# apapiu/transformer_latent_diffusion

Hardware: AMD Instinct MI355X
Metric: images/sec (256px, 35-step CFG sampling), denoiser only (higher is better)
Workload: dtype bf16; 1 GPU; C1: 100M-param denoiser (d=768, L=12), 32x32x4 latents, 35 steps + CFG 6, DPM-Solver++(2M), 64 images/GPU (model batch 128); images_per_gpu=64, global_batch=64, n_iter=35, parallelism=single GPU

## Files before the change

### transformer_latent_diffusion_amd/csrc/tld_common.h

```cpp
#pragma once
#include <hip/hip_runtime.h>
#include <atomic>
#include <mutex>
#include <stdint.h>
#include "tld_gemm_plan.h"

namespace tld {

typedef __attribute__((ext_vector_type(8))) __bf16 bf16x8;
typedef __attribute__((ext_vector_type(4))) __bf16 bf16x4;
typedef __attribute__((ext_vector_type(2))) __bf16 bf16x2;
typedef __attribute__((ext_vector_type(16))) float f32x16;
typedef __attribute__((ext_vector_type(4))) float f32x4;
typedef __attribute__((ext_vector_type(4))) unsigned u32x4;
typedef __attribute__((ext_vector_type(8))) int i32x8;
typedef __attribute__((ext_vector_type(2))) float f32x2;

constexpr int kWave = 64;
constexpr int kHeadDim = 64;
constexpr float kLnEps = 1e-5f;

template <int CTRL>
__device__ __forceinline__ float dpp_add(float v) {
    const int s = __builtin_amdgcn_update_dpp(0, __float_as_int(v), CTRL, 0xf, 0xf, true);
// ... 185 lines not shown
    std::mutex mu;
    template <class F> void run(int want, F&& set_attribute) {
        int dev = 0;
        (void)hipGetDevice(&dev);
        std::atomic<int>& a = v[dev & 63];
        if (a.load(std::memory_order_acquire) >= want) return;
        std::lock_guard<std::mutex> lk(mu);
        if (a.load(std::memory_order_relaxed) >= want) return;
        set_attribute();
        a.store(want, std::memory_order_release);
    }
};
inline int ptr_device(const void* p) {
    hipPointerAttribute_t a;
    if (p && hipPointerGetAttributes(&a, p) == hipSuccess) return a.device;
    (void)hipGetLastError();
    return -1;
}
struct PtrDeviceGuard {
    int prev = -1; bool switched = false;
    explicit PtrDeviceGuard(const void* p) {
        const int dev = ptr_device(p);
        if (dev >= 0 && hipGetDevice(&prev) == hipSuccess && prev != dev) switched = hipSetDevice(dev) == hipSuccess;
    }
    ~PtrDeviceGuard() { if (switched) (void)hipSetDevice(prev); }
    PtrDeviceGuard(const PtrDeviceGuard&) = delete;
    PtrDeviceGuard& operator=(const PtrDeviceGuard&) = delete;
};
inline int device_cu_count() {
    static int cus[64] = {0};
    int dev = 0;
    (void)hipGetDevice(&dev);
    int& c = cus[dev & 63];
    if (!c) {
        int n = 0;
        if (hipDeviceGetAttribute(&n, hipDeviceAttributeMultiprocessorCount, dev) != hipSuccess || n <= 0) n = 256;
        c = n;
    }
    return c;
}

enum : int {
    EP_EMBED_PLAIN = 0, EP_EMBED_MFMA = 1 , EP_LN_Q4 = 5 , EP_LN_GENERIC = 9, EP_LN_MX8 = 10,
    EP_QKV_ATTN = 11, EP_QKV_LN = 12, EP_QKV_PLAIN = 13,
    EP_ATT_256 = 14, EP_ATT_CHUNKED = 15, EP_ATT_64 = 17 , EP_ATT_MASKED = 19,
    EP_CROSS_MFMA = 20 , EP_CROSS_GPW1 = 24, EP_CROSS_GPWN = 25, EP_CROSS_VALU = 26, EP_CROSS_FANOUT = 27,
    EP_UP_FUSED16 = 28, EP_UP_FUSED32_SEAM = 29, EP_UP_FUSED16_SMALL = 30, EP_UP_PLAIN = 31, EP_DW_WHOLE = 32, EP_DW_TILED = 33, EP_DW_STREAM = 34,
    EP_DOWN_STATS = 35, EP_DOWN_NOSTATS = 36, EP_DOWN_MAIN = 37, EP_DOWN_SMALL64 = 38, EP_DOWN_SMALL128 = 39,
    EP_SPLITK4 = 40, EP_SPLITK8 = 41, EP_SPLITK_SMALL = 42, EP_SPLITK_FINISH12 = 43, EP_SPLITK_FINISH6 = 44,
    EP_TAIL_MFMA = 45 , EP_TAIL_PLAIN = 49, EP_UPDATE = 50, EP_UPDATE_FROM = 51, EP_UPDATE_FROM_MASK = 52, EP_START_MIX = 53,
    EP_QUANT_MX8 = 54, EP_CROSS_F8 = 55, EP_DW_TILED_F8 = 56, EP_DW_STREAM_F8 = 57,
    EP_UPDATE_REQ = 58, EP_UPDATE_REQ_MASK = 59, EP_START_MIX_REQ = 60,
    EP_TAIL_FOLD = 16,
    EP_COUNT = 61
};
extern thread_local uint64_t* g_path_sink;
inline void note_path(int bit) { if (g_path_sink) *g_path_sink |= 1ull << bit; }

int launch_gemm(const GemmParams& p, int epilogue, hipStream_t s);
void launch_updw_pp(const GemmParams& p, const GemmPlan& plan, hipStream_t s);
void launch_splitk_pp(const GemmParams& p, const GemmPlan& plan, hipStream_t s);
void launch_down_pp(const GemmParams& p, const GemmPlan& plan, hipStream_t s);
void launch_dwconv_seam(const uint32_t* seam, const uint32_t* dw_wpk, const float* dw_b_half, bf16* out, int ldo, int batch, int channels, hipStream_t s);
void launch_gemm_tn(const GemmParams& p, hipStream_t s);

void set_last_error(const char* msg);

void launch_quant_mx8(const bf16* in, uint8_t* out, uint8_t* scale, int M, int K, hipStream_t s);
void quant_mx8_host(const float* w, int rows, int K, uint8_t* out, uint8_t* scale);

void launch_attention(const bf16* qk, const bf16* vt, bf16* att, int batch, int ntok, int heads,
                      hipStream_t s);

void launch_dwconv_gelu(const bf16* in, bf16* out, const float* w9c , const float* bias, const float* w9c_half,
                        const float* bias_half, int batch, int grid, int channels, hipStream_t s, uint8_t* out8 = nullptr,
                        uint8_t* scale8 = nullptr);

struct EmbedParams {
    const float* x;
    const float* conv_w;
    const float* conv_b;
    const float* ln1_w; const float* ln1_b;
    const float* lin_wt;
    const bf16* lin_w_hl;
    const float* lin_b;
    const float* ln2_w; const float* ln2_b;
    const float* pos;
    resid_t* tok;
    float2* stats_out;
    int batch, src_batch;
    const int* src_row;
    int C, S, p, grid, pd, d, ntok;
};
void launch_embed(const EmbedParams& p, hipStream_t s);

void launch_layernorm_bf16(const resid_t* x, const float* g, const float* b, bf16* out, int M, int d,
                           hipStream_t s);
bool layernorm_mx8_supported(int d);
void launch_layernorm_mx8(const resid_t* x, const float* g, const float* b, uint8_t* out8, uint8_t* scale8, int M, int d,
                          hipStream_t s);

struct CrossRowParams {
    resid_t* x;
    const resid_t* x_in;
    const bf16* att;
    int src_batch;
// ... 76 lines not shown
```

### transformer_latent_diffusion_amd/csrc/tld_cond.hip

```cpp
#include "tld_common.h"
#include <hip/hip_fp16.h>

namespace tld {

namespace {

__global__ void sinusoid_kernel(const float* __restrict__ sigma, const float* __restrict__ angular,
                                float* __restrict__ out, int T, int half) {
    const int i = blockIdx.x * blockDim.x + threadIdx.x;
    if (i >= T * half) return;
    const int t = i / half, k = i - t * half;
    const float ph = angular[k] * sigma[t];
    out[(size_t)t * 2 * half + k] = sinf(ph);
    out[(size_t)t * 2 * half + half + k] = cosf(ph);
}

constexpr int LR = 8;
__global__ __launch_bounds__(256) void linear_f32_kernel(const float* __restrict__ in, int ldi,
                                                         const float* __restrict__ W,
                                                         const float* const* __restrict__ Wl,
                                                         const float* __restrict__ bias,
                                                         float* __restrict__ out, size_t out_lstride, int ldo, int T,
                                                         int K, int N, int act) {
    if (Wl) { W = Wl[blockIdx.z]; out += (size_t)blockIdx.z * out_lstride; }
    extern __shared__ __attribute__((aligned(16))) char smem[];
    float* xs = reinterpret_cast<float*>(smem);
    const int t0 = blockIdx.y * LR;
    for (int i = threadIdx.x; i < LR * K; i += 256) {
        const int r = i / K, k = i - r * K;
        const int t = t0 + r;
        xs[i] = t < T ? in[(size_t)t * ldi + k] : 0.f;
    }
    __syncthreads();
    const int lane = threadIdx.x & 63, wid = threadIdx.x >> 6;
    for (int c = 0; c < 16; ++c) {
        const int n = blockIdx.x * 64 + wid * 16 + c;
        if (n >= N) break;
        float acc[LR];
#pragma unroll
        for (int r = 0; r < LR; ++r) acc[r] = 0.f;
        const float* wrow = W + (size_t)n * K;
        for (int k = lane; k < K; k += 64) {
            const float w = wrow[k];
#pragma unroll
            for (int r = 0; r < LR; ++r) acc[r] += xs[r * K + k] * w;
        }
#pragma unroll
        for (int r = 0; r < LR; ++r) acc[r] = wave_sum(acc[r]);
        if (lane < LR) {
            float v = 0.f;
#pragma unroll
            for (int r = 0; r < LR; ++r) if (lane == r) v = acc[r];
            const int t = t0 + lane;
            if (t < T) {
                v += bias ? bias[n] : 0.f;
                if (act == 1) v = gelu_erf(v);
                out[(size_t)t * ldo + n] = v;
            }
        }
    }
}

__global__ __launch_bounds__(256) void layernorm_f32_kernel(const float* __restrict__ x,
                                                            const float* __restrict__ g,
                                                            const float* __restrict__ b,
                                                            float* __restrict__ out, int M, int d) {
    const int lane = threadIdx.x & 63;
    const int row = blockIdx.x * 4 + (threadIdx.x >> 6);
    if (row >= M) return;
    float s = 0.f;
    for (int k = lane; k < d; k += 64) s += x[(size_t)row * d + k];
    const float mean = wave_sum(s) / (float)d;
    float q = 0.f;
    for (int k = lane; k < d; k += 64) { const float c = x[(size_t)row * d + k] - mean; q += c * c; }
    const float rstd = 1.0f / sqrtf(wave_sum(q) / (float)d + kLnEps);
    for (int k = lane; k < d; k += 64)
        out[(size_t)row * d + k] = (x[(size_t)row * d + k] - mean) * rstd * g[k] + b[k];
}

__global__ __launch_bounds__(256) void wq_kernel(const float* __restrict__ kmat, size_t k_lstride, int ldk,
                                                 const float* const* __restrict__ Wql,
                                                 const float* const* __restrict__ gammal,
                                                 const float* const* __restrict__ betal, float* __restrict__ wq,
                                                 size_t wq_lstride, float* __restrict__ bwq, size_t bwq_lstride, int T,
                                                 int H, int d) {
    const float* __restrict__ Wq = Wql[blockIdx.z];
    const float* __restrict__ gamma = gammal[blockIdx.z];
    const float* __restrict__ beta = betal[blockIdx.z];
    kmat += (size_t)blockIdx.z * k_lstride; wq += (size_t)blockIdx.z * wq_lstride; bwq += (size_t)blockIdx.z * bwq_lstride;
    __shared__ float ks[LR][64];
    __shared__ float red[4][LR];
    const int h = blockIdx.x, t0 = blockIdx.y * LR;
    for (int i = threadIdx.x; i < LR * 64; i += 256) {
        const int r = i >> 6, c = i & 63;
        const int t = t0 + r;
        ks[r][c] = t < T ? kmat[(size_t)t * ldk + h * 64 + c] * 0.125f : 0.f;
    }
    __syncthreads();
    float bacc[LR];
#pragma unroll
    for (int r = 0; r < LR; ++r) bacc[r] = 0.f;
    for (int j = threadIdx.x; j < d; j += 256) {
        float acc[LR];
#pragma unroll
        for (int r = 0; r < LR; ++r) acc[r] = 0.f;
        for (int c = 0; c < 64; ++c) {
            const float w = Wq[(size_t)(h * 64 + c) * d + j];
#pragma unroll
            for (int r = 0; r < LR; ++r) acc[r] += ks[r][c] * w;
        }
        const float gj = gamma[j], bj = beta[j];
#pragma unroll
        for (int r = 0; r < LR; ++r) {
            const int t = t0 + r;
            if (t < T) wq[((size_t)t * H + h) * d + j] = acc[r] * gj;
            bacc[r] += acc[r] * bj;
        }
    }
    const int lane = threadIdx.x & 63, wid = threadIdx.x >> 6;
#pragma unroll
    for (int r = 0; r < LR; ++r) {
        const float tot = wave_sum(bacc[r]);
        if (lane == 0) red[wid][r] = tot;
    }
    __syncthreads();
    if (threadIdx.x < LR) {
        const int t = t0 + threadIdx.x;
        if (t < T) bwq[(size_t)t * H + h] = red[0][threadIdx.x] + red[1][threadIdx.x] + red[2][threadIdx.x] + red[3][threadIdx.x];
    }
}

__global__ void iota_kernel(int* __restrict__ dst, int n, int base) {
    const int i = blockIdx.x * blockDim.x + threadIdx.x;
    if (i < n) dst[i] = base + i;
}

__global__ void fill_bf16_kernel(bf16* __restrict__ dst, int64_t n, uint32_t seed, float scale) {
    const int64_t i = (int64_t)blockIdx.x * blockDim.x + threadIdx.x;
    if (i >= n) return;
    uint32_t h = (uint32_t)i * 2654435761u + seed;
    h ^= h >> 15; h *= 2246822519u; h ^= h >> 13; h *= 3266489917u; h ^= h >> 16;
    dst[i] = (bf16)(((float)(h >> 8) * (1.0f / 8388608.0f) - 1.0f) * scale);
}

template <typename T>
__global__ void cast_to_f32_kernel(const T* __restrict__ src, float* __restrict__ dst, int64_t n) {
    const int64_t i = (int64_t)blockIdx.x * blockDim.x + threadIdx.x;
    if (i < n) dst[i] = (float)src[i];
}
template <typename T>
__global__ void cast_from_f32_kernel(const float* __restrict__ src, T* __restrict__ dst, int64_t n) {
    const int64_t i = (int64_t)blockIdx.x * blockDim.x + threadIdx.x;
    if (i < n) dst[i] = (T)src[i];
}

}

void launch_sinusoid(const float* sigma, const float* angular, float* out, int T, int half, hipStream_t s) {
    const int n = T * half;
    hipLaunchKernelGGL(sinusoid_kernel, dim3((n + 255) / 256), dim3(256), 0, s, sigma, angular, out, T, half);
}

void launch_linear_f32(const float* in, int ldi, const float* W, const float* b, float* out, int ldo, int T,
                       int K, int N, int act, hipStream_t s) {
    dim3 grid((N + 63) / 64, (T + LR - 1) / LR);
    hipLaunchKernelGGL(linear_f32_kernel, grid, dim3(256), LR * K * sizeof(float), s, in, ldi, W,
                       (const float* const*)nullptr, b, out, (size_t)0, ldo, T, K, N, act);
}

void launch_linear_f32_layers(const float* in, int ldi, const float* const* Wl, float* out, size_t out_lstride,
                              int ldo, int T, int K, int N, int layers, hipStream_t s) {
    dim3 grid((N + 63) / 64, (T + LR - 1) / LR, layers);
    hipLaunchKernelGGL(linear_f32_kernel, grid, dim3(256), LR * K * sizeof(float), s, in, ldi, (const float*)nullptr,
                       Wl, (const float*)nullptr, out, out_lstride, ldo, T, K, N, 0);
}

void launch_layernorm_f32(const float* x, const float* g, const float* b, float* out, int M, int d,
                          hipStream_t s) {
    hipLaunchKernelGGL(layernorm_f32_kernel, dim3((M + 3) / 4), dim3(256), 0, s, x, g, b, out, M, d);
}

void launch_wq_layers(const float* k, size_t k_lstride, int ldk, const float* const* Wql, const float* const* gammal,
                      const float* const* betal, float* wq, size_t wq_lstride, float* bwq, size_t bwq_lstride, int T,
                      int heads, int d, int layers, hipStream_t s) {
    dim3 grid(heads, (T + LR - 1) / LR, layers);
    hipLaunchKernelGGL(wq_kernel, grid, dim3(256), 0, s, k, k_lstride, ldk, Wql, gammal, betal, wq, wq_lstride, bwq,
                       bwq_lstride, T, heads, d);
}

void launch_iota(int* dst, int n, int base, hipStream_t s) {
    hipLaunchKernelGGL(iota_kernel, dim3((n + 255) / 256), dim3(256), 0, s, dst, n, base);
}

void launch_fill_bf16(bf16* dst, int64_t n, uint32_t seed, float scale, hipStream_t s) {
    hipLaunchKernelGGL(fill_bf16_kernel, dim3((unsigned)((n + 255) / 256)), dim3(256), 0, s, dst, n, seed, scale);
}

void launch_cast_to_f32(const void* src, int dtype, float* dst, int64_t n, hipStream_t s) {
    dim3 grid((unsigned)((n + 255) / 256)), block(256);
    if (dtype == 1) hipLaunchKernelGGL(cast_to_f32_kernel<bf16>, grid, block, 0, s, (const bf16*)src, dst, n);
    else if (dtype == 2) hipLaunchKernelGGL(cast_to_f32_kernel<__half>, grid, block, 0, s, (const __half*)src, dst, n);
    else hipMemcpyAsync(dst, src, n * sizeof(float), hipMemcpyDeviceToDevice, s);
}

void launch_cast_from_f32(const float* src, void* dst, int dtype, int64_t n, hipStream_t s) {
    dim3 grid((unsigned)((n + 255) / 256)), block(256);
    if (dtype == 1) hipLaunchKernelGGL(cast_from_f32_kernel<bf16>, grid, block, 0, s, src, (bf16*)dst, n);
    else if (dtype == 2) hipLaunchKernelGGL(cast_from_f32_kernel<__half>, grid, block, 0, s, src, (__half*)dst, n);
    else hipMemcpyAsync(dst, src, n * sizeof(float), hipMemcpyDeviceToDevice, s);
}

}
```

### transformer_latent_diffusion_amd/csrc/tld_rows.hip

```cpp
#include "tld_common.h"
#include <cstdlib>

namespace tld {

namespace {


template <int NJ, bool HALF>
__global__ __launch_bounds__(256) void embed_kernel(EmbedParams p) {
    extern __shared__ __attribute__((aligned(16))) char smem[];
    constexpr int d = NJ * 128 - (HALF ? 64 : 0);
    float* wt = reinterpret_cast<float*>(smem);
    float* cwt = wt + p.pd * d;
    for (int i = threadIdx.x; i < p.pd * d / 4; i += 256)
        reinterpret_cast<float4*>(wt)[i] = reinterpret_cast<const float4*>(p.lin_wt)[i];
    for (int i = threadIdx.x; i < p.pd * p.C * p.p * p.p; i += 256) {
        const int o = i / (p.C * p.p * p.p), k = i - o * (p.C * p.p * p.p);
        cwt[k * p.pd + o] = p.conv_w[i];
    }
    __syncthreads();
    const int lane = threadIdx.x & 63;
    const int wid = __builtin_amdgcn_readfirstlane(threadIdx.x >> 6);
    const bool live_last = !HALF || lane < 32;
    auto live = [&](int j) { return j + 1 < NJ || live_last; };
    const int pp = p.p * p.p, cpp = p.C * pp;
    const int total = p.batch * p.ntok;
    const float cb = lane < p.pd ? p.conv_b[lane] : 0.f;
    const float* cw = cwt + (lane < p.pd ? lane : 0);
    const float g1 = lane < p.pd ? p.ln1_w[lane] : 0.f, b1 = lane < p.pd ? p.ln1_b[lane] : 0.f;
    const int ic = lane / pp, iuv = lane - ic * pp, iu = iuv / p.p, iv = iuv - iu * p.p;
    constexpr int ROWS_PER_WAVE = 8;
    auto load_in = [&](int row) {
        float xv = 0.f;
        if (row < total && lane < cpp) {
            const int b = row / p.ntok, t = row - b * p.ntok;
            const int ti = t / p.grid, tj = t - ti * p.grid;
            xv = p.x[(((size_t)(p.src_row ? p.src_row[b] : b % p.src_batch) * p.C + ic) * p.S + (ti * p.p + iu)) * p.S + (tj * p.p + iv)];
        }
        return xv;
    };
    const int row_first = (blockIdx.x * 4 + wid) * ROWS_PER_WAVE;
    float xnext = load_in(row_first);
    for (int rr = 0; rr < ROWS_PER_WAVE; ++rr) {
        const int row = row_first + rr;
        if (row >= total) return;
        const int t = row % p.ntok;
        const float xin = xnext;
        if (rr + 1 < ROWS_PER_WAVE) xnext = load_in(row + 1);
        float pv = cb;
        {
            int i = 0;
            for (; i + 4 <= cpp; i += 4) {
                const float c0 = cw[(i + 0) * p.pd], c1 = cw[(i + 1) * p.pd], c2 = cw[(i + 2) * p.pd], c3 = cw[(i + 3) * p.pd];
                pv = fmaf(c0, __int_as_float(__builtin_amdgcn_readlane(__float_as_int(xin), i + 0)), pv);
// ... 901 lines not shown
    };
    auto mma = [&](int buf, int kb0) {
#pragma unroll
        for (int g = 0; g < G; ++g) {
            if (kb0 + g < kb_hi) {
#pragma unroll
                for (int rt = 0; rt < RT; ++rt)
#pragma unroll
                    for (int t = 0; t < NT; ++t) acc[rt][t] = __builtin_amdgcn_mfma_f32_16x16x32_bf16(wh[buf][g][t], xa[buf][g][rt], acc[rt][t], 0, 0, 0);
#pragma unroll
                for (int rt = 0; rt < RT; ++rt)
#pragma unroll
                    for (int t = 0; t < NT; ++t) acc[rt][t] = __builtin_amdgcn_mfma_f32_16x16x32_bf16(wl[buf][g][t], xa[buf][g][rt], acc[rt][t], 0, 0, 0);
            }
        }
    };
    fetch(0, kb_lo);
    for (int kb0 = kb_lo; kb0 < kb_hi; kb0 += 2 * G) {
        fetch(1, kb0 + G);
        __builtin_amdgcn_sched_barrier(0);
        mma(0, kb0);
        __builtin_amdgcn_sched_barrier(0);
        fetch(0, kb0 + 2 * G);
        __builtin_amdgcn_sched_barrier(0);
        mma(1, kb0 + G);
        __builtin_amdgcn_sched_barrier(0);
    }
#pragma unroll
    for (int rt = 0; rt < RT; ++rt)
#pragma unroll
        for (int t = 0; t < NT; ++t) red[(wid * (RT * NT) + rt * NT + t) * 64 + lane] = acc[rt][t];
    __syncthreads();
    const int pp = p.p * p.p;
    for (int it = wid; it < RT * NT; it += 8) {
        const int rt = it / NT, t = it - rt * NT;
        f32x4 s[8];
#pragma unroll
        for (int w = 0; w < 8; ++w) s[w] = red[(w * (RT * NT) + it) * 64 + lane];
        const f32x4 sum = ((s[0] + s[1]) + (s[2] + s[3])) + ((s[4] + s[5]) + (s[6] + s[7]));
        const int row = row0 + rt * 16 + tok;
        if (row >= total) continue;
        const int b = row / p.ntok, tk = row - b * p.ntok;
        const int ti = tk / p.grid, tj = tk - ti * p.grid;
#pragma unroll
        for (int r = 0; r < 4; ++r) {
            const int f = t * 16 + 4 * kq + r;
            if (f < p.pd) {
                const int c = f / pp, uv = f - c * pp;
                const int u = uv / p.p, vv = uv - u * p.p;
                p.out[(((size_t)b * p.C + c) * p.S + (ti * p.p + u)) * p.S + (tj * p.p + vv)] = sum[r] + p.bf[f];
            }
        }
    }
}

__global__ __launch_bounds__(256) void tail_fold_debug_row_kernel(float* __restrict__ row, const bf16* __restrict__ x, const float* __restrict__ bias, int64_t n, int d) {
    const int64_t i = (int64_t)blockIdx.x * 256 + threadIdx.x;
    if (i < n) row[i] = ((float)x[i] + row[i]) + bias[(int)(i % d)];
}
#endif

template <bool MASK, int V, bool SLOT = false>
__global__ __launch_bounds__(256) void sampler_step_kernel(SamplerStepParams p) {
#pragma clang fp contract(off)
    const int i = (blockIdx.x * 256 + threadIdx.x) * V;
    const int n = p.active * p.img;
    if (i >= n) return;
    float cond[V], unc[V], prev[V], xin[V], eps[V], z[V], m[V], x0o[V], xto[V];
    auto load = [&](float* dst, const float* src) {
        if constexpr (V == 4) *reinterpret_cast<float4*>(dst) = *reinterpret_cast<const float4*>(src);
        else dst[0] = src[0];
    };
    auto store = [&](float* dst, const float* src) {
        if constexpr (V == 4) *reinterpret_cast<float4*>(dst) = *reinterpret_cast<const float4*>(src);
        else dst[0] = src[0];
    };
    const int b = i / p.img, r = i - b * p.img;
    const int ch = r / p.chan_stride;
    const SamplerStepRow q = p.rows[b * p.row_stride];
    load(cond, p.x0_2b + i);
    const int slot = SLOT ? (q.final_step >> 1) - 1 : 0;
    const bool final_step = SLOT ? (q.final_step & 1) != 0 : q.final_step != 0;
    if constexpr (SLOT) {
        if (slot >= 0) load(unc, p.x0_2b + (size_t)(p.active + slot) * p.img + r);
    } else {
        load(unc, p.x0_2b + n + i);
    }
    auto combine = [&](float c, float u) {
        if constexpr (SLOT) { if (slot < 0) return c; }
        return __builtin_fmaf(q.g, c, (1.0f - q.g) * u);
    };
    if constexpr (MASK) {
        load(m, p.mask + (size_t)b * p.chan_stride + (r - ch * p.chan_stride));
        load(z, p.z0 + i);
    }
    if (final_step) {
#pragma unroll
        for (int v = 0; v < V; ++v) {
            float x0 = combine(cond[v], unc[v]);
            if constexpr (MASK) x0 = m[v] * x0 + (1.0f - m[v]) * z[v];
            if (ch == 3) x0 += p.sharp;
            if (ch == 0) x0 += p.bright;
            x0o[v] = x0;
        }
        store(p.out_latent + i, x0o);
        return;
// ... 323 lines not shown

template <int CPL>
__global__ __launch_bounds__(256) void splitk_resid_kernel(const float* __restrict__ parts, int nsplit, size_t slice_stride, const float* __restrict__ bias,
                                                           resid_t* __restrict__ x, float2* __restrict__ stats_out, int M) {
    constexpr int d = CPL * 64, GL = 96 / CPL;
    static_assert(96 % CPL == 0 && (GL & (GL - 1)) == 0 && CPL % 2 == 0, "a 96-column group must be a power-of-two run of lanes");
    const int lane = threadIdx.x & 63;
    const int row = blockIdx.x * 4 + (threadIdx.x >> 6);
    if (row >= M) return;
    float v[CPL];
#pragma unroll
    for (int c = 0; c < CPL; c += 2) {
        const float2 b2 = *reinterpret_cast<const float2*>(bias + CPL * lane + c);
        v[c] = b2.x; v[c + 1] = b2.y;
    }
    for (int sp = 0; sp < nsplit; ++sp) {
        const float* src = parts + sp * slice_stride + (size_t)row * d + CPL * lane;
#pragma unroll
        for (int c = 0; c < CPL; c += 2) {
            const float2 t = *reinterpret_cast<const float2*>(src + c);
            v[c] += t.x; v[c + 1] += t.y;
        }
    }
    resid_t* px = x + (size_t)row * d + CPL * lane;
    float su = 0.f, sq = 0.f;
#pragma unroll
    for (int c = 0; c < CPL; c += 2) {
        const float2 xv = rs_load2(px + c);
        const float o0 = xv.x + v[c], o1 = xv.y + v[c + 1];
        rs_store2(px + c, make_float2(o0, o1));
        const float r0 = rs_round(o0), r1 = rs_round(o1);
        su += r0 + r1;
        sq = fmaf(r0, r0, fmaf(r1, r1, sq));
    }
    if (stats_out) {
#pragma unroll
        for (int o2 = 1; o2 < GL; o2 <<= 1) { su += __shfl_xor(su, o2, 64); sq += __shfl_xor(sq, o2, 64); }
        const int slot = lane / GL;
        if ((lane & (GL - 1)) == 0 && slot < kLnSlots) stats_out[(size_t)row * kLnSlots + slot] = make_float2(su, sq);
    }
}

bool splitk_resid_supported(int d) { return d == 768 || d == 384; }

void launch_splitk_resid(const float* parts, int nsplit, size_t slice_stride, const float* bias, resid_t* x, float2* stats_out, int M, int d, hipStream_t s) {
    const dim3 grid((unsigned)((M + 3) / 4)), block(256);
    if (d == 768) { note_path(EP_SPLITK_FINISH12); hipLaunchKernelGGL(splitk_resid_kernel<12>, grid, block, 0, s, parts, nsplit, slice_stride, bias, x, stats_out, M); }
    else if (d == 384) { note_path(EP_SPLITK_FINISH6); hipLaunchKernelGGL(splitk_resid_kernel<6>, grid, block, 0, s, parts, nsplit, slice_stride, bias, x, stats_out, M); }
}

void launch_tail(const TailParams& p, hipStream_t s) {
#ifdef TLD_RESID_BF16
    if (p.hid) {
        const int nt = (p.pd + 15) / 16, rows = p.batch * p.ntok;
        const int big = nt <= 2 ? 4 : 2;
        const int rt = rows >= 16 * big * device_cu_count() ? big : 1;
        const int lds = 8 * rt * nt * 1024;
        dim3 grid((unsigned)((rows + 16 * rt - 1) / (16 * rt)));
#define TLD_TF(NT, RT) hipLaunchKernelGGL((tail_fold_kernel<NT, RT>), grid, dim3(512), lds, s, p)
        note_path(EP_TAIL_MFMA + nt - 1); note_path(EP_TAIL_FOLD);
        if (nt == 1) { if (rt == 1) TLD_TF(1, 1); else TLD_TF(1, 4); }
        else if (nt == 2) { if (rt == 1) TLD_TF(2, 1); else TLD_TF(2, 4); }
        else if (nt == 3) { if (rt == 1) TLD_TF(3, 1); else TLD_TF(3, 2); }
        else { if (rt == 1) TLD_TF(4, 1); else TLD_TF(4, 2); }
#undef TLD_TF
        return;
    }
    if (p.w_hl && p.d % 128 == 0 && (long)p.pd * p.d <= 40960) {
        const int nt = (p.pd + 15) / 16, rows = p.batch * p.ntok;
        const int lds = 2 * nt * 16 * p.d * 2;
        dim3 grid((unsigned)((rows + 63) / 64));
#define TLD_TM(NT) do { TLD_LDS_OPT_IN((tail_mfma_kernel<NT>), lds); hipLaunchKernelGGL((tail_mfma_kernel<NT>), grid, dim3(256), lds, s, p, p.w_hl); } while (0)
        note_path(EP_TAIL_MFMA + (nt < 4 ? nt : 4) - 1);
        if (nt == 1) TLD_TM(1); else if (nt == 2) TLD_TM(2); else if (nt == 3) TLD_TM(3); else TLD_TM(4);
#undef TLD_TM
        return;
    }
#endif
    const int rpb = 64;
    const int rows = p.batch * p.ntok;
    const int lds = p.pd * p.d * (int)sizeof(float);
    note_path(EP_TAIL_PLAIN);
    TLD_DISPATCH_D(p.d, { TLD_LDS_OPT_IN((tail_kernel<NJ, HALF>), lds); hipLaunchKernelGGL((tail_kernel<NJ, HALF>), dim3((rows + rpb - 1) / rpb), dim3(256), lds, s, p, rpb); });
}

#ifdef TLD_RESID_BF16
void launch_tail_fold_debug_row(float* row, const resid_t* x, const float* bias, int M, int d, hipStream_t s) {
    const int64_t n = (int64_t)M * d;
    hipLaunchKernelGGL(tail_fold_debug_row_kernel, dim3((unsigned)((n + 255) / 256)), dim3(256), 0, s, row, x, bias, n, d);
}
#endif

namespace {
bool aligned16(const void* a) { return (reinterpret_cast<uintptr_t>(a) & 15) == 0; }
}

void launch_sampler_step(const SamplerStepParams& p, int path, hipStream_t s, bool slots) {
    const int n = p.active * p.img;
    const bool vec = p.img % 4 == 0 && p.chan_stride % 4 == 0 && aligned16(p.x0_2b) && aligned16(p.x_t) && aligned16(p.x0_prev) && aligned16(p.out_latent) &&
                     aligned16(p.trace_x0) && aligned16(p.trace_xt) && aligned16(p.noise) && aligned16(p.z0) && aligned16(p.mask);
    const int threads = vec ? n / 4 : n;
    const dim3 grid((threads + 255) / 256), block(256);
    note_path(path);
    if (slots) {
        if (p.mask) {
            if (vec) hipLaunchKernelGGL((sampler_step_kernel<true, 4, true>), grid, block, 0, s, p);
            else hipLaunchKernelGGL((sampler_step_kernel<true, 1, true>), grid, block, 0, s, p);
        } else {
            if (vec) hipLaunchKernelGGL((sampler_step_kernel<false, 4, true>), grid, block, 0, s, p);
            else hipLaunchKernelGGL((sampler_step_kernel<false, 1, true>), grid, block, 0, s, p);
        }
    } else if (p.mask) {
        if (vec) hipLaunchKernelGGL((sampler_step_kernel<true, 4>), grid, block, 0, s, p);
// ... 242 lines not shown
```

### transformer_latent_diffusion_amd/denoiser.py

```python
from __future__ import annotations

import ctypes as C
import os
from collections import OrderedDict
from typing import Dict, Iterator, Optional

import numpy as np
import torch

from . import _lib
from .weights import param_count, param_layout, state_dict_spec, synth_state_dict

_IO_DTYPES = {torch.float32: _lib.DTYPE_F32, torch.bfloat16: _lib.DTYPE_BF16, torch.float16: _lib.DTYPE_F16}


class Denoiser:
    def __init__(self, image_size: int, noise_embed_dims: int, patch_size: int, embed_dim: int, dropout: float,
                 n_layers: int, text_emb_size: int = 768, mlp_multiplier: int = 4, n_channels: int = 4,
                 init_seed: int = 0):
        self.image_size = image_size
        self.noise_embed_dims = noise_embed_dims
        self.patch_size = patch_size
        self.embed_dim = embed_dim
        self.dropout = dropout
# ... 324 lines not shown
            raise ValueError("init_latents is required with a mask or with a start_mix < 1")
        neg, has_neg = None, [False] * B
        if neg_labels is not None:
            if isinstance(neg_labels, torch.Tensor):
                if tuple(neg_labels.shape) != (B, self.text_emb_size):
                    raise ValueError(f"neg_labels {tuple(neg_labels.shape)}: expected {(B, self.text_emb_size)}")
                neg, has_neg = neg_labels, [True] * B
            else:
                rows = list(neg_labels)
                if len(rows) != B:
                    raise ValueError(f"neg_labels: {len(rows)} entries for {B} requests")
                for b, r in enumerate(rows):
                    if r is not None and tuple(r.shape) != (self.text_emb_size,):
                        raise ValueError(f"neg_labels[{b}] {tuple(r.shape)}: expected {(self.text_emb_size,)}")
                has_neg = [r is not None for r in rows]
                if any(has_neg):
                    dev = self._resolve_device(noise)
                    neg = torch.stack([torch.zeros(self.text_emb_size, device=dev) if r is None else r.detach().to(dev, torch.float32) for r in rows])
        counts = [t.shape[0] for t in tabs]
        order = schedule.request_order(counts)
        n_max = counts[order[0]] if B else 0
        rows_needed = schedule.request_cond_rows([tabs[b] for b in order], sum(has_neg)) if B else 0
        if rows_needed > schedule.REQUEST_ROW_CAP:
            raise ValueError(f"the call needs {rows_needed} conditioning rows (distinct noise levels + labels): at most {schedule.REQUEST_ROW_CAP}")
        table = np.zeros((B, n_max, 6), dtype=np.float32)
        recs = (_lib.TldSampleRequest * B)()
        for k, b in enumerate(order):
            table[k, :counts[b]] = tabs[b]
            recs[k] = _lib.TldSampleRequest(counts[b], guid[b], mix[b], int(has_neg[b]))
        if steps is not None:
            gtab = np.zeros((B, n_max), dtype=np.float32)
            for k, b in enumerate(order):
                gtab[k, :counts[b]] = steps[b]

            def model_batch(skip):
                if not B:
                    return 0
                sc = [counts[b] for b in order]
                U = schedule.guided_rows(sc, [steps[b] for b in order], skip)[0]
                return max(bi + u for bi, u in zip(schedule.active_prefix(sc), U))

            return self._run_sampler(noise, labels, n_max, trace, lambda h, B, eps, z0, m, lab, ng, out, tx0, txt, stream: _lib.check(
                _lib.lib().tld_sample_requests_guided(h, eps, z0, m, lab, ng, recs, table.ctypes.data_as(C.POINTER(C.c_float)),
                                                      gtab.ctypes.data_as(C.POINTER(C.c_float)), n_max, float(sharp_f), float(bright_f), out, B, tx0,
                                                      txt, stream), "tld_sample_requests_guided"),
                init_latents=init_latents, mask=mask, neg_labels=neg, order=order, new_trace=torch.zeros, model_batch=model_batch)
        return self._run_sampler(noise, labels, n_max, trace, lambda h, B, eps, z0, m, lab, ng, out, tx0, txt, stream: _lib.check(
            _lib.lib().tld_sample_requests(h, eps, z0, m, lab, ng, recs, table.ctypes.data_as(C.POINTER(C.c_float)), n_max, float(sharp_f),
                                           float(bright_f), out, B, tx0, txt, stream), "tld_sample_requests"),
            init_latents=init_latents, mask=mask, neg_labels=neg, order=order, new_trace=torch.zeros)

    PATH_NAMES = ("embed plain", "embed_mfma<2>", "embed_mfma<4>", "embed_mfma<6>", "embed_mfma<8>", "layernorm q4<1>", "layernorm q4<2>", "layernorm q4<3>",
                  "layernorm q4<4>", "layernorm generic", "layernorm mx8", "QKV fused with attention", "QKV LayerNorm-1 fold", "QKV plain", "attention 256",
                  "attention chunked", "tail folded", "attention 64", None, "attention masked", "cross_row_mfma<1>", "cross_row_mfma<2>",
                  "cross_row_mfma<3>", "cross_row_mfma<4>", "cross_row gpw 1", "cross_row gpw > 1", "cross_row VALU", "cross_row x_in fan-out",
                  "up fused 16", "up fused 32 + seam", "up fused 16 4-wave", "up alone", "depthwise whole image", "depthwise tiled", "depthwise streaming",
                  "down with stats_out", "down without stats_out", "down 8-wave", "down 4-wave 64", "down 4-wave 128", "split-K x4", "split-K x8",
                  "split-K 4-wave", "split-K finisher<12>", "split-K finisher<6>", "tail_mfma<1>", "tail_mfma<2>", "tail_mfma<3>", "tail_mfma<4>", None,
                  "update", "update_from", "update_from masked", "start_mix")
    FP8_PATH_NAMES = {10: "layernorm mx8", 54: "fp8 separate quantisation pass", 55: "fp8 cross_row writer", 56: "fp8 depthwise tiled",
                      57: "fp8 depthwise streaming"}

    SAMPLER_PATH_NAMES = {58: "update_requests", 59: "update_requests masked", 60: "start_mix per request"}

    def sample_rows(self):
        c, u = C.c_int64(), C.c_int64()
        _lib.check(_lib.lib().tld_engine_sample_rows(self._engine, C.byref(c), C.byref(u)), "tld_engine_sample_rows")
        return int(c.value), int(u.value)

    def set_debug(self, enable: bool = True):
        _lib.check(_lib.lib().tld_engine_set_debug(self._engine, int(enable)), "tld_engine_set_debug")

    def set_debug_step(self, step: int):
        _lib.check(_lib.lib().tld_engine_set_debug_step(self._engine, int(step)), "tld_engine_set_debug_step")

    def debug_paths(self) -> int:
        m = C.c_uint64()
        _lib.check(_lib.lib().tld_engine_debug_paths(self._engine, C.byref(m)), "tld_engine_debug_paths")
        return int(m.value)

    def stage_shape(self, name: str):
        sh = (C.c_int64 * 4)()
        _lib.check(_lib.lib().tld_engine_stage_shape(self._engine, name.encode(), sh), f"tld_engine_stage_shape({name})")
        sh = list(sh)
        while len(sh) > 1 and sh[-1] == 1:
            sh.pop()
        return tuple(sh)

    def read_stage(self, name: str, shape=None) -> np.ndarray:
        out = np.empty(self.stage_shape(name) if shape is None else shape, dtype=np.float32)
        _lib.check(_lib.lib().tld_engine_read_stage(self._engine, name.encode(),
                                                    out.ctypes.data_as(C.POINTER(C.c_float)), out.size),
                   f"tld_engine_read_stage({name})")
        return out

    def set_profile(self, classes=()):
        mask = 0
        for c in classes:
            mask |= 1 << _lib.KERNEL_CLASSES.index(c)
        _lib.check(_lib.lib().tld_engine_set_profile(self._engine, mask), "tld_engine_set_profile")

    def reserve_profile(self, cls: str, launches: int):
        _lib.check(_lib.lib().tld_engine_profile_reserve(self._engine, _lib.KERNEL_CLASSES.index(cls), int(launches)),
                   "tld_engine_profile_reserve")

    def get_profile(self, cls: str):
        ms, n = C.c_double(), C.c_int64()
# ... 4 lines not shown
```

Measured before the change: 305.8 images/s.

## Add persistent streaming tail-fold kernel and MFMA f32 conditioning linear

Adds a persistent tail-fold kernel. Each workgroup keeps its slice of the folded output-projection weights (bf16 hi/lo split) in registers and streams row groups with prefetched inputs and double-buffered LDS reduction, replacing one launch tile per row group when there are enough rows. It also routes the f32 conditioning linears to an MFMA 16x16x4 f32 kernel with software prefetch when alignment allows, instead of the VALU wave-reduction kernel. The aim is to cut weight reloads and launch or tail overhead in the final projection and to speed up the conditioning MLPs, at the cost of higher register pressure and more code paths.

```diff
diff --git a/transformer_latent_diffusion_amd/csrc/tld_common.h b/transformer_latent_diffusion_amd/csrc/tld_common.h
--- a/transformer_latent_diffusion_amd/csrc/tld_common.h
+++ b/transformer_latent_diffusion_amd/csrc/tld_common.h
@@ -261,6 +261,7 @@
     EP_QUANT_MX8 = 54, EP_CROSS_F8 = 55, EP_DW_TILED_F8 = 56, EP_DW_STREAM_F8 = 57,
     EP_UPDATE_REQ = 58, EP_UPDATE_REQ_MASK = 59, EP_START_MIX_REQ = 60,
     EP_TAIL_FOLD = 16,
+    EP_TAIL_STREAM = 18,
     EP_COUNT = 61
 };
 extern thread_local uint64_t* g_path_sink;
diff --git a/transformer_latent_diffusion_amd/csrc/tld_cond.hip b/transformer_latent_diffusion_amd/csrc/tld_cond.hip
--- a/transformer_latent_diffusion_amd/csrc/tld_cond.hip
+++ b/transformer_latent_diffusion_amd/csrc/tld_cond.hip
@@ -59,6 +59,69 @@
             }
         }
     }
+}
+
+template <int RT>
+__global__ __launch_bounds__(256) void linear_f32_mfma_kernel(const float* __restrict__ in, int ldi, const float* __restrict__ W,
+                                                              const float* const* __restrict__ Wl, const float* __restrict__ bias,
+                                                              float* __restrict__ out, size_t out_lstride, int ldo, int T, int K, int N, int act) {
+    if (Wl) { W = Wl[blockIdx.z]; out += (size_t)blockIdx.z * out_lstride; }
+    const int lane = threadIdx.x & 63, wid = __builtin_amdgcn_readfirstlane(threadIdx.x >> 6);
+    const int r = lane & 15, kq = lane >> 4;
+    const int n0 = blockIdx.x * 64 + wid * 16;
+    if (n0 >= N) return;
+    const int t0 = blockIdx.y * (16 * RT);
+    typedef const float __attribute__((address_space(1))) gfloat;
+    gfloat* wp = (gfloat*)W + (size_t)(n0 + r) * K + kq * 4;
+    const float* xp[RT];
+#pragma unroll
+    for (int rt = 0; rt < RT; ++rt) {
+        const int t = t0 + rt * 16 + r;
+        xp[rt] = in + (size_t)(t < T ? t : T - 1) * ldi + kq * 4;
+    }
+    f32x4 acc[RT];
+#pragma unroll
+    for (int rt = 0; rt < RT; ++rt) acc[rt] = f32x4{0.f, 0.f, 0.f, 0.f};
+    constexpr int PF = 4;
+    const int nks = K >> 4;
+    f32x4 wf[PF], xf[PF][RT];
+#pragma unroll
+    for (int i = 0; i < PF; ++i) {
+        wf[i] = *(const f32x4 __attribute__((address_space(1)))*)(wp + i * 16);
+#pragma unroll
+        for (int rt = 0; rt < RT; ++rt) xf[i][rt] = *reinterpret_cast<const f32x4*>(xp[rt] + i * 16);
+    }
+    for (int ks0 = 0; ks0 < nks; ks0 += PF) {
+#pragma unroll
+        for (int i = 0; i < PF; ++i) {
+            const f32x4 wv = wf[i];
+            f32x4 xv[RT];
+#pragma unroll
+            for (int rt = 0; rt < RT; ++rt) xv[rt] = xf[i][rt];
+            const int nk = ks0 + i + PF < nks ? ks0 + i + PF : nks - 1;
+            wf[i] = *(const f32x4 __attribute__((address_space(1)))*)(wp + nk * 16);
+#pragma unroll
+            for (int rt = 0; rt < RT; ++rt) xf[i][rt] = *reinterpret_cast<const f32x4*>(xp[rt] + nk * 16);
+#pragma unroll
+            for (int j = 0; j < 4; ++j)
+#pragma unroll
+                for (int rt = 0; rt < RT; ++rt) acc[rt] = __builtin_amdgcn_mfma_f32_16x16x4f32(xv[rt][j], wv[j], acc[rt], 0, 0, 0);
+            __builtin_amdgcn_sched_barrier(0);
+        }
+    }
+    const int n = n0 + r;
+    const float bn = bias ? bias[n] : 0.f;
+#pragma unroll
+    for (int rt = 0; rt < RT; ++rt)
+#pragma unroll
+        for (int q = 0; q < 4; ++q) {
+            const int t = t0 + rt * 16 + kq * 4 + q;
+            if (t < T) {
+                float v = acc[rt][q] + bn;
+                if (act == 1) v = gelu_erf(v);
+                out[(size_t)t * ldo + n] = v;
+            }
+        }
 }
 
 __global__ __launch_bounds__(256) void layernorm_f32_kernel(const float* __restrict__ x,
@@ -161,18 +224,33 @@
     hipLaunchKernelGGL(sinusoid_kernel, dim3((n + 255) / 256), dim3(256), 0, s, sigma, angular, out, T, half);
 }
 
+namespace {
+void launch_linear(const float* in, int ldi, const float* W, const float* const* Wl, const float* b, float* out, size_t out_lstride, int ldo, int T, int K,
+                   int N, int act, int layers, hipStream_t s) {
+    if (T <= 0 || N <= 0) return;
+    const bool mfma = K > 0 && K % 64 == 0 && N % 16 == 0 && ldi % 4 == 0 && (reinterpret_cast<uintptr_t>(in) & 15) == 0 &&
+                      (Wl || (reinterpret_cast<uintptr_t>(W) & 15) == 0);
+    if (mfma) {
+        const int rt = T <= 16 ? 1 : T <= 32 ? 2 : 4;
+        dim3 grid((N + 63) / 64, (T + 16 * rt - 1) / (16 * rt), layers);
+#define TLD_LIN(RT) hipLaunchKernelGGL((linear_f32_mfma_kernel<RT>), grid, dim3(256), 0, s, in, ldi, W, Wl, b, out, out_lstride, ldo, T, K, N, act)
+        if (rt == 1) TLD_LIN(1); else if (rt == 2) TLD_LIN(2); else TLD_LIN(4);
+#undef TLD_LIN
+        return;
+    }
+    dim3 grid((N + 63) / 64, (T + LR - 1) / LR, layers);
+    hipLaunchKernelGGL(linear_f32_kernel, grid, dim3(256), LR * K * sizeof(float), s, in, ldi, W, Wl, b, out, out_lstride, ldo, T, K, N, act);
+}
+}
+
 void launch_linear_f32(const float* in, int ldi, const float* W, const float* b, float* out, int ldo, int T,
                        int K, int N, int act, hipStream_t s) {
-    dim3 grid((N + 63) / 64, (T + LR - 1) / LR);
-    hipLaunchKernelGGL(linear_f32_kernel, grid, dim3(256), LR * K * sizeof(float), s, in, ldi, W,
-                       (const float* const*)nullptr, b, out, (size_t)0, ldo, T, K, N, act);
+    launch_linear(in, ldi, W, nullptr, b, out, 0, ldo, T, K, N, act, 1, s);
 }
 
 void launch_linear_f32_layers(const float* in, int ldi, const float* const* Wl, float* out, size_t out_lstride,
                               int ldo, int T, int K, int N, int layers, hipStream_t s) {
-    dim3 grid((N + 63) / 64, (T + LR - 1) / LR, layers);
-    hipLaunchKernelGGL(linear_f32_kernel, grid, dim3(256), LR * K * sizeof(float), s, in, ldi, (const float*)nullptr,
-                       Wl, (const float*)nullptr, out, out_lstride, ldo, T, K, N, 0);
+    launch_linear(in, ldi, nullptr, Wl, nullptr, out, out_lstride, ldo, T, K, N, 0, layers, s);
 }
 
 void launch_layernorm_f32(const float* x, const float* g, const float* b, float* out, int M, int d,
diff --git a/transformer_latent_diffusion_amd/csrc/tld_rows.hip b/transformer_latent_diffusion_amd/csrc/tld_rows.hip
--- a/transformer_latent_diffusion_amd/csrc/tld_rows.hip
+++ b/transformer_latent_diffusion_amd/csrc/tld_rows.hip
@@ -1,5 +1,7 @@
 #include "tld_common.h"
+#include "tld_tail_plan.h"
 #include <cstdlib>
+#include <type_traits>
 
 namespace tld {
 
@@ -1007,6 +1009,104 @@
             }
         }
     }
+}
+
+template <int PER, int RT, bool FULL>
+__global__ __launch_bounds__(512) void tail_stream_kernel(TailParams p, int ngroups) {
+    extern __shared__ __attribute__((aligned(16))) char smem[];
+    f32x4* red = reinterpret_cast<f32x4*>(smem);
+    const int d = p.d, K = d + p.hidn;
+    const int lane = threadIdx.x & 63, wid = __builtin_amdgcn_readfirstlane(threadIdx.x >> 6);
+    const int tok = lane & 15, kq = lane >> 4;
+    const int total = p.batch * p.ntok;
+    const int nkb = K >> 5, dkb = d >> 5;
+    const int per = (nkb + 7) >> 3;
+    const int kb_lo = wid * per, kb_hi = kb_lo + per < nkb ? kb_lo + per : nkb;
+    const int G = gridDim.x;
+    bf16x8 wh[PER], wl[PER];
+    {
+        const bf16* wbase = p.wf_hl + (size_t)tok * K + kq * 8;
+        const size_t lo_plane = (size_t)16 * K;
+#pragma unroll
+        for (int j = 0; j < PER; ++j) {
+            const int kb = kb_lo + j < nkb ? kb_lo + j : nkb - 1;
+            wh[j] = *reinterpret_cast<const bf16x8*>(wbase + kb * 32);
+            wl[j] = *reinterpret_cast<const bf16x8*>(wbase + lo_plane + kb * 32);
+        }
+    }
+    auto row_offsets = [&](int g, int rt, unsigned& xo, unsigned& ho) {
+        const int r = (g * RT + rt) * 16 + tok;
+        const unsigned row = (unsigned)(r < total ? r : total - 1);
+        xo = row * (unsigned)d + kq * 8; ho = row * (unsigned)p.hidn + kq * 8;
+    };
+    auto load = [&](int j, unsigned xo, unsigned ho) {
+        const int kb = kb_lo + j < nkb ? kb_lo + j : nkb - 1;
+        const bool in_x = kb < dkb;
+        const int ko = (in_x ? kb : kb - dkb) * 32;
+        return *reinterpret_cast<const bf16x8*>(in_x ? p.tok + xo + ko : p.hid + ho + ko);
+    };
+    bf16x8 xa[PER];
+    int g = blockIdx.x;
+    {
+        unsigned xo, ho;
+        row_offsets(g, 0, xo, ho);
+#pragma unroll
+        for (int j = 0; j < PER; ++j) xa[j] = load(j, xo, ho);
+    }
+    static_assert(RT == 4, "one (tile, feature pair) per wave");
+    const int srt = wid >> 1, part = wid & 1;
+    float sbias[2];
+    int soff[2];
+#pragma unroll
+    for (int r = 0; r < 2; ++r) {
+        const int f = 4 * kq + 2 * part + r, pp = p.p * p.p;
+        const int c = f / pp, uv = f - c * pp;
+        const int u = uv / p.p, vv = uv - u * p.p;
+        sbias[r] = f < p.pd ? p.bf[f] : 0.f;
+        soff[r] = f < p.pd ? (c * p.S + u) * p.S + vv : -1;
+    }
+    int buf = 0;
+    auto group = [&](auto last) {
+        constexpr bool LAST = decltype(last)::value;
+        f32x4* rb = red + buf * (8 * RT * 64);
+#pragma unroll
+        for (int rt = 0; rt < RT; ++rt) {
+            f32x4 acc = f32x4{0.f, 0.f, 0.f, 0.f};
+            const bool more = rt + 1 < RT || !LAST;
+            unsigned xo = 0, ho = 0;
+            if (more) { if (rt + 1 < RT) row_offsets(g, rt + 1, xo, ho); else row_offsets(g + G, 0, xo, ho); }
+#pragma unroll
+            for (int j = 0; j < PER; ++j) {
+                const bf16x8 xb = xa[j];
+                if (more) xa[j] = load(j, xo, ho);
+                if (FULL || kb_lo + j < kb_hi) {
+                    acc = __builtin_amdgcn_mfma_f32_16x16x32_bf16(wh[j], xb, acc, 0, 0, 0);
+                    acc = __builtin_amdgcn_mfma_f32_16x16x32_bf16(wl[j], xb, acc, 0, 0, 0);
+                }
+                __builtin_amdgcn_sched_barrier(0);
+            }
+            rb[(wid * RT + rt) * 64 + lane] = acc;
+        }
+        __syncthreads();
+        {
+            float2 s[8];
+#pragma unroll
+            for (int w = 0; w < 8; ++w) s[w] = *(reinterpret_cast<const float2*>(rb + (w * RT + srt) * 64 + lane) + part);
+            const int row = (g * RT + srt) * 16 + tok;
+            if (row < total) {
+                const int b = row / p.ntok, tk = row - b * p.ntok;
+                const int ti = tk / p.grid, tj = tk - ti * p.grid;
+                float* o = p.out + ((size_t)b * p.C * p.S + ti * p.p) * p.S + tj * p.p;
+                const float sum0 = ((s[0].x + s[1].x) + (s[2].x + s[3].x)) + ((s[4].x + s[5].x) + (s[6].x + s[7].x));
+                const float sum1 = ((s[0].y + s[1].y) + (s[2].y + s[3].y)) + ((s[4].y + s[5].y) + (s[6].y + s[7].y));
+                if (soff[0] >= 0) o[soff[0]] = sum0 + sbias[0];
+                if (soff[1] >= 0) o[soff[1]] = sum1 + sbias[1];
+            }
+        }
+        buf ^= 1;
+    };
+    for (; g + G < ngroups; g += G) group(std::false_type{});
+    group(std::true_type{});
 }
 
 __global__ __launch_bounds__(256) void tail_fold_debug_row_kernel(float* __restrict__ row, const bf16* __restrict__ x, const float* __restrict__ bias, int64_t n, int d) {
@@ -1436,13 +1536,23 @@
 void launch_tail(const TailParams& p, hipStream_t s) {
 #ifdef TLD_RESID_BF16
     if (p.hid) {
-        const int nt = (p.pd + 15) / 16, rows = p.batch * p.ntok;
-        const int big = nt <= 2 ? 4 : 2;
-        const int rt = rows >= 16 * big * device_cu_count() ? big : 1;
-        const int lds = 8 * rt * nt * 1024;
-        dim3 grid((unsigned)((rows + 16 * rt - 1) / (16 * rt)));
+        const int rows = p.batch * p.ntok;
+        static const bool stream_on = [] { const char* e = getenv("TLD_TAIL_STREAM"); return !e || atoi(e) != 0; }();
+        const TailPlan plan = plan_tail_fold(rows, p.pd, p.d, p.hidn, device_cu_count(), stream_on);
+        const int nt = plan.nt, rt = plan.rt, lds = plan.lds;
+        dim3 grid((unsigned)plan.grid);
+        note_path(EP_TAIL_MFMA + nt - 1); note_path(EP_TAIL_FOLD);
+        if (plan.form == TAIL_FORM_STREAM) {
+            const int ngroups = (rows + 16 * rt - 1) / (16 * rt);
+            note_path(EP_TAIL_STREAM);
+#define TLD_TS(PER, FULL) hipLaunchKernelGGL((tail_stream_kernel<PER, kTailStreamRt, FULL>), grid, dim3(512), lds, s, p, ngroups)
+            if (plan.per == 15) TLD_TS(15, true);
+            else if (plan.per == 8) TLD_TS(8, false);
+            else TLD_TS(4, false);
+#undef TLD_TS
+            return;
+        }
 #define TLD_TF(NT, RT) hipLaunchKernelGGL((tail_fold_kernel<NT, RT>), grid, dim3(512), lds, s, p)
-        note_path(EP_TAIL_MFMA + nt - 1); note_path(EP_TAIL_FOLD);
         if (nt == 1) { if (rt == 1) TLD_TF(1, 1); else TLD_TF(1, 4); }
         else if (nt == 2) { if (rt == 1) TLD_TF(2, 1); else TLD_TF(2, 4); }
         else if (nt == 3) { if (rt == 1) TLD_TF(3, 1); else TLD_TF(3, 2); }
diff --git a/transformer_latent_diffusion_amd/csrc/tld_tail_plan.h b/transformer_latent_diffusion_amd/csrc/tld_tail_plan.h
--- /dev/null
+++ b/transformer_latent_diffusion_amd/csrc/tld_tail_plan.h
@@ -0,0 +1,52 @@
+#pragma once
+
+namespace tld {
+
+enum TailForm { TAIL_FORM_TILES = 0, TAIL_FORM_STREAM = 1 };
+
+struct TailPlan {
+    int form;
+    int nt;
+    int rt;
+    int per;
+    int full;
+    int grid;
+    int lds;
+    int wregs;
+};
+
+constexpr int kTailWaves = 8;
+constexpr int kTailStreamRt = 4;
+constexpr int kTailStreamMaxWregs = 120;
+constexpr int kTailLdsLimit = 64 * 1024;
+
+constexpr int tail_stream_per(int nkb) {
+    const int per = (nkb + kTailWaves - 1) / kTailWaves;
+    return per <= 4 ? 4 : per <= 8 ? 8 : nkb == 15 * kTailWaves ? 15 : 0;
+}
+
+inline TailPlan plan_tail_fold(long rows, int pd, int d, int hid, int cus, bool allow_stream = true) {
+    TailPlan t{};
+    t.nt = (pd + 15) / 16;
+    const int nkb = (d + hid) / 32;
+    const int big = t.nt <= 2 ? 4 : 2;
+    const int per = t.nt == 1 ? tail_stream_per(nkb) : 0;
+    if (allow_stream && per && 8 * per * t.nt <= kTailStreamMaxWregs && rows >= 16L * kTailStreamRt * cus) {
+        const long groups = (rows + 16 * kTailStreamRt - 1) / (16 * kTailStreamRt);
+        t.form = TAIL_FORM_STREAM;
+        t.rt = kTailStreamRt;
+        t.per = per;
+        t.full = nkb == kTailWaves * per;
+        t.grid = (int)(groups < cus ? groups : cus);
+        t.lds = 2 * kTailWaves * t.rt * 1024;
+        t.wregs = 8 * per * t.nt;
+        return t;
+    }
+    t.form = TAIL_FORM_TILES;
+    t.rt = rows >= 16L * big * cus ? big : 1;
+    t.grid = (int)((rows + 16 * t.rt - 1) / (16 * t.rt));
+    t.lds = kTailWaves * t.rt * t.nt * 1024;
+    return t;
+}
+
+}
diff --git a/transformer_latent_diffusion_amd/denoiser.py b/transformer_latent_diffusion_amd/denoiser.py
--- a/transformer_latent_diffusion_amd/denoiser.py
+++ b/transformer_latent_diffusion_amd/denoiser.py
@@ -400,7 +400,7 @@
 
     PATH_NAMES = ("embed plain", "embed_mfma<2>", "embed_mfma<4>", "embed_mfma<6>", "embed_mfma<8>", "layernorm q4<1>", "layernorm q4<2>", "layernorm q4<3>",
                   "layernorm q4<4>", "layernorm generic", "layernorm mx8", "QKV fused with attention", "QKV LayerNorm-1 fold", "QKV plain", "attention 256",
-                  "attention chunked", "tail folded", "attention 64", None, "attention masked", "cross_row_mfma<1>", "cross_row_mfma<2>",
+                  "attention chunked", "tail folded", "attention 64", "tail folded streaming", "attention masked", "cross_row_mfma<1>", "cross_row_mfma<2>",
                   "cross_row_mfma<3>", "cross_row_mfma<4>", "cross_row gpw 1", "cross_row gpw > 1", "cross_row VALU", "cross_row x_in fan-out",
                   "up fused 16", "up fused 32 + seam", "up fused 16 4-wave", "up alone", "depthwise whole image", "depthwise tiled", "depthwise streaming",
                   "down with stats_out", "down without stats_out", "down 8-wave", "down 4-wave 64", "down 4-wave 128", "split-K x4", "split-K x8",
```

Result: no change. 307.8 images/s, median of 6 (+0.6%).
